# jbelyeu/unfazed

Hardware: AMD Instinct MI355X
Metric: phased DNMs/sec (higher is better)
Workload: dtype u8/int32 (+f64 allele balance); 1 GPU; 100k synthetic SNV/INDEL DNMs, whole-genome sites VCF, --no-extended off (BASELINE configs[2]); staged: H2D of the pre-decoded columns inside the timed region; dnms_per_gpu=100000, sites=20000000, coverage=30x, search_dist=5000, dnm_placement=uniform, read_clusters=67821, alignment_records=186931612, parallelism=dnm-shard x1, no collective

## Files before the change

### include/unfazed_io.h

```cpp
#ifndef UNFAZED_IO_H
#define UNFAZED_IO_H
#include <stdint.h>
#include "uz_types.h"
#include "uz_bamwalk.h"

#ifdef __cplusplus
extern "C" {
#endif

#define UZ_IO_OK 0
#define UZ_IO_E_OPEN (-1)
#define UZ_IO_E_FORMAT (-2)
#define UZ_IO_E_UNSORTED (-3)
#define UZ_IO_E_RANGE (-4)
#define UZ_IO_E_ARG (-5)

const char *uz_io_last_error(void);

typedef struct uz_bam uz_bam;

int uz_bam_decode(const char *path, int threads, uz_bam **out);
int uz_bam_decode_regions(const char *path, const char *bai_path, int64_t n_iv, const int32_t *tid, const int32_t *lo, const int32_t *hi,
                          int64_t head_records, int threads, uz_bam **out);
int uz_bam_decode_memory(const uint8_t *stream, int64_t n, int threads, uz_bam **out);
// ... 33 lines not shown
int uz_vcf_decode_regions(const char *path, const char *tbi_path, int64_t n_iv, const int32_t *ref, const int32_t *lo, const int32_t *hi,
                          int threads, uz_vcf **out);
int64_t uz_vcf_index_names(const char *path, const char *tbi_path, char *buf, int64_t cap);
int64_t uz_index_summary(const char *path, int kind, int64_t *out, int64_t cap_refs);
void uz_vcf_io_stats(const uz_vcf *h, int64_t out[4]);
void uz_vcf_free(uz_vcf *h);
int uz_vcf_view_get(const uz_vcf *h, uz_vcf_view *out);
const char *uz_vcf_sample(const uz_vcf *h, int32_t i);
const char *uz_vcf_contig(const uz_vcf *h, int32_t i);
const char *uz_vcf_ref(const uz_vcf *h, int64_t i, int32_t *len);
const char *uz_vcf_alt(const uz_vcf *h, int64_t i, int32_t *len);
const char *uz_vcf_header(const uz_vcf *h, int64_t *len);
const char *uz_vcf_line(const uz_vcf *h, int64_t i, int32_t *len);
const char *uz_vcf_info(const uz_vcf *h, int64_t i, const char *key, int32_t *len);
int uz_vcf_is_bcf(const uz_vcf *h);

int uz_reads_pack_sizes(const uz_reads_view *in, int64_t *n_cigar_total, int64_t *n_row_units);
int uz_reads_pack_cigar_omitted(const uz_reads_view *in, int threads, int64_t *n_omitted);
int uz_reads_pack_end_derivable(const uz_reads_view *in, int threads, int32_t *yes);
int uz_reads_pack_lists(const uz_reads_view *in, int min_base_qual, int threads, int64_t *n_qlow_pos, int32_t *wide);
int uz_reads_pack_exceptions(const uz_reads_view *in, int threads, int64_t *n_exc);
int uz_reads_pack(const uz_reads_view *in, int min_base_qual, int threads, uz_reads_packed_view *out);

typedef struct uz_psrc uz_psrc;
typedef struct uz_select uz_select;
int uz_reads_source_open(const uz_reads_packed_view *full, int threads, uz_psrc **out);
void uz_reads_source_close(uz_psrc *src);
int uz_reads_select_plan(const uz_psrc *src, int64_t n_fetch, const int32_t *contig, const int32_t *lo, const int32_t *hi, int all_bases,
                         int unit_masks, const uint16_t *extra, int tuples, int threads, uz_select **out);
int64_t uz_select_n_tuples(const uz_select *s);
// ... 82 lines not shown
```

### include/uz_types.h

```cpp
#ifndef UZ_TYPES_H
#define UZ_TYPES_H

#include <stdint.h>

#ifdef __cplusplus
extern "C" {
#endif

#define UZ_HOM_REF 0
#define UZ_HET 1
#define UZ_GT_UNKNOWN 2
#define UZ_HOM_ALT 3

#define UZ_U16_MISSING 0xFFFFu

#define UZ_SF_COMPLEX 1u

#define UZ_CL_HET 0x01u
#define UZ_CL_CAND 0x02u
#define UZ_CL_ALT_DAD 0x04u
#define UZ_CL_DEL_SHIFT 3
#define UZ_CL_DUP_SHIFT 5
#define UZ_KA_NONE 0
#define UZ_KA_REF_PARENT 1
// ... 48 lines not shown
    int32_t reserved0;
    double ab_homref[2];
    double ab_homalt[2];
    double ab_het[2];
} uz_params;

typedef struct uz_sites_view {
    int64_t n_sites;
    int32_t n_contigs;
    int32_t reserved0;
    const int64_t *contig_off;
    const int32_t *pos;
    const uint8_t *sflags;
    const uint8_t *ref_base;
    const uint8_t *alt_base;
} uz_sites_view;

typedef struct uz_family_view {
    const uint8_t *gt;
    const uint16_t *ref_depth[3];
    const uint16_t *alt_depth[3];
    const uint16_t *gq[3];
    int64_t n_wide;
    const int64_t *wide_site;
    const int32_t *wide_ref_depth[3];
    const int32_t *wide_alt_depth[3];
    const uint8_t *ref_depth8[3];
    const uint8_t *alt_depth8[3];
    const uint8_t *gq8[3];
} uz_family_view;
#define UZ_U8_MISSING 254u
// ... 153 lines not shown
```

### unfazed_amd/abi.py

```python
from __future__ import annotations

import ctypes as C
from typing import List, Optional, Sequence

import numpy as np

from .model import ReadsTable, SitesTable

ST_OK, ST_NO_CAND, ST_NO_OVERLAP, ST_REF_EXCEPTION, ST_SKIPPED, ST_CAPACITY = 0, 1, 2, 3, 4, 5
OR_NONE, OR_DAD, OR_MOM, OR_AMBIGUOUS = 0, 1, 2, 3
VT_POINT, VT_DEL, VT_DUP, VT_OTHER_SV = 0, 1, 2, 3
DF_FETCH_FALLBACK = 1
CF_ALT_DAD = 1
CF_KA_SHIFT = 1
CL_HET, CL_CAND, CL_ALT_DAD = 1, 2, 4
CL_DEL_SHIFT, CL_DUP_SHIFT = 3, 5
ET_READBACKED, ET_ALLELE_BALANCE, ET_AMBIGUOUS_READBACKED, ET_AMBIGUOUS_ALLELE_BALANCE, ET_AMBIGUOUS_BOTH, ET_AMBIG_FLAG = 1, 2, 4, 8, 16, 32
ET_NAMES = [(ET_READBACKED, "READBACKED"), (ET_AMBIGUOUS_READBACKED, "AMBIGUOUS_READBACKED"), (ET_ALLELE_BALANCE, "ALLELE-BALANCE"),
            (ET_AMBIGUOUS_ALLELE_BALANCE, "AMBIGUOUS_ALLELE-BALANCE"), (ET_AMBIGUOUS_BOTH, "AMBIGUOUS_BOTH")]
FIND_WHOLE_REGION = 1
FIND_SECOND_WINDOW = 2

_p = C.c_void_p

# ... 44 lines not shown
    p.ab_homalt[0], p.ab_homalt[1] = float(ab_homalt[0]), float(ab_homalt[1])
    p.ab_het[0], p.ab_het[1] = float(ab_het[0]), float(ab_het[1])
    return p


class SitesView(C.Structure):
    _fields_ = [
        ("n_sites", C.c_int64),
        ("n_contigs", C.c_int32),
        ("reserved0", C.c_int32),
        ("contig_off", _p),
        ("pos", _p),
        ("sflags", _p),
        ("ref_base", _p),
        ("alt_base", _p),
    ]


class FamilyView(C.Structure):
    _fields_ = [
        ("gt", _p),
        ("ref_depth", _p * 3),
        ("alt_depth", _p * 3),
        ("gq", _p * 3),
        ("n_wide", C.c_int64),
        ("wide_site", _p),
        ("wide_ref_depth", _p * 3),
        ("wide_alt_depth", _p * 3),
        ("ref_depth8", _p * 3),
        ("alt_depth8", _p * 3),
# ... 529 lines not shown
```

### unfazed_amd/csrc/abi.hip

```cpp
#include "uz_ctx.hpp"

#include <chrono>
#include <algorithm>
#include <map>
#include <mutex>

void uz_fold_complex(uz_ctx *c, uint8_t *gt, const uint8_t *sflags, int64_t n);
bool uz_site_scan_fresh(const uz_ctx *c, const FamilyDev &f, bool need_cnv);

namespace {

void set_error(uz_ctx *c, const std::string &msg) {
    std::lock_guard<std::mutex> lk(c->err_mu);
    c->err = msg;
}

template <typename F>
int guarded(uz_ctx *c, F &&fn) {
    if (!c) return UZ_E_ARG;
    try {
        (void)hipSetDevice(c->device);
        fn();
        return 0;
    } catch (const UzError &e) {
// ... 89 lines not shown
template <typename V>
int new_slot(std::vector<V> &v) {
    for (size_t i = 0; i < v.size(); i++)
        if (!v[i].live) return (int)i;
    v.emplace_back();
    return (int)v.size() - 1;
}

SitesDev &sites_of(uz_ctx *c, int id) {
    UZ_REQUIRE(id >= 0 && id < (int)c->sites.size() && c->sites[id].live, UZ_E_ARG, "unknown sites handle");
    SitesDev &s = c->sites[id];
    if (s.pending) {
        s.pending = false;
        UZ_HIP(hipStreamWaitEvent(c->stream, s.ready, 0));
    }
    return s;
}
FamilyDev &fam_of(uz_ctx *c, int id) {
    UZ_REQUIRE(id >= 0 && id < (int)c->fams.size() && c->fams[id].live, UZ_E_ARG, "unknown family handle");
    FamilyDev &f = c->fams[id];
    if (f.pending) {
        f.pending = false;
        UZ_HIP(hipStreamWaitEvent(c->stream, f.ready, 0));
        SitesDev &s = sites_of(c, f.sites_id);
        uz_family_widen(c, f, s.n);
        uz_fold_complex(c, f.gt, s.sflags, s.n);
    }
    return f;
}
ReadsDev &reads_of(uz_ctx *c, int id) {
    UZ_REQUIRE(id >= 0 && id < (int)c->reads.size() && c->reads[id].live, UZ_E_ARG, "unknown reads handle");
    return c->reads[id];
}

void free_family(uz_ctx *c, FamilyDev &f) {
    if (f.ready) { (void)hipEventSynchronize(f.ready); (void)hipEventDestroy(f.ready); f.ready = nullptr; }
    f.pending = false;
    uz_block_put(c, f.block);
    uz_block_put(c, f.wide_block);
    f = FamilyDev();
}
// ... 284 lines not shown

int uz_sync(uz_ctx *c) {
    return guarded(c, [&] { UZ_HIP(hipStreamSynchronize(c->stream)); });
}

int uz_set_params(uz_ctx *c, const uz_params *p) {
    return guarded(c, [&] {
        UZ_REQUIRE(p != nullptr, UZ_E_ARG, "null params");
        c->P = *p;
    });
}

int uz_sites_upload(uz_ctx *c, const uz_sites_view *v, int *id) {
    return guarded(c, [&] {
        UZ_REQUIRE(v && id && v->n_sites >= 0 && v->n_contigs >= 0, UZ_E_ARG, "bad sites view");
        UZ_REQUIRE(v->n_sites < (int64_t)0x7FFFFFF0, UZ_E_RANGE, "more than 2^31 sites");
        const int k = new_slot(c->sites);
        SitesDev s;
        s.live = true; s.owned = true;
        s.n = v->n_sites; s.n_contigs = v->n_contigs;
        s.contig_off_h.assign(v->contig_off, v->contig_off + v->n_contigs + 1);
        const size_t n = (size_t)s.n;
        for (int pass = 0; pass < 2; pass++) {
            Carver cv(pass ? s.block.p : nullptr);
            s.contig_off = cv.take<int64_t>((size_t)v->n_contigs + 1);
            s.pos = cv.take<int32_t>(n); s.sflags = cv.take<uint8_t>(n); s.ref_base = cv.take<uint8_t>(n); s.alt_base = cv.take<uint8_t>(n);
            if (!pass) s.block = uz_block_get(c, cv.off + 256);
        }
        try {
            h2d(c->stream, s.contig_off, v->contig_off, (size_t)v->n_contigs + 1);
            h2d(c->stream, s.pos, v->pos, n); h2d(c->stream, s.sflags, v->sflags, n);
            h2d(c->stream, s.ref_base, v->ref_base, n); h2d(c->stream, s.alt_base, v->alt_base, n);
            UZ_HIP(hipStreamSynchronize(c->stream));
        } catch (...) { uz_block_put(c, s.block); throw; }
        c->sites[k] = s;
        *id = k;
    });
}

int uz_sites_adopt_device(uz_ctx *c, const uz_sites_view *v, int *id) {
    return guarded(c, [&] {
        UZ_REQUIRE(v && id && v->n_sites >= 0 && v->n_contigs >= 0, UZ_E_ARG, "bad sites view");
        const int k = new_slot(c->sites);
        SitesDev s;
        s.live = true; s.owned = false;
        s.n = v->n_sites; s.n_contigs = v->n_contigs;
        s.contig_off_h.resize((size_t)v->n_contigs + 1);
        UZ_HIP(hipMemcpy(s.contig_off_h.data(), v->contig_off, ((size_t)v->n_contigs + 1) * sizeof(int64_t), hipMemcpyDeviceToHost));
        for (int pass = 0; pass < 2; pass++) {
            Carver cv(pass ? s.block.p : nullptr);
            s.contig_off = cv.take<int64_t>((size_t)v->n_contigs + 1);
            if (!pass) s.block = uz_block_get(c, cv.off + 256);
        }
        h2d(c->stream, s.contig_off, (const int64_t *)s.contig_off_h.data(), (size_t)v->n_contigs + 1);
        s.pos = const_cast<int32_t *>(v->pos);
        s.sflags = const_cast<uint8_t *>(v->sflags);
        s.ref_base = const_cast<uint8_t *>(v->ref_base);
        s.alt_base = const_cast<uint8_t *>(v->alt_base);
        UZ_HIP(hipStreamSynchronize(c->stream));
        c->sites[k] = s;
        *id = k;
    });
}

static bool family_view_eight(const uz_family_view *v) {
    int n8 = 0, n16 = 0;
    for (int m = 0; m < 3; m++) {
        n8 += (v->ref_depth8[m] != nullptr) + (v->alt_depth8[m] != nullptr) + (v->gq8[m] != nullptr);
        n16 += (v->ref_depth[m] != nullptr) + (v->alt_depth[m] != nullptr) + (v->gq[m] != nullptr);
    }
    UZ_REQUIRE((n8 == 9 && n16 == 0) || (n8 == 0 && n16 == 9) || (n8 == 0 && n16 == 0), UZ_E_ARG,
               "a family view carries its nine columns in 16 bits OR in 8 bits (ref_depth8 / alt_depth8 / gq8), all nine");
    return n8 == 9;
}

static void family_wide(uz_ctx *c, hipStream_t st, const uz_family_view *v, FamilyDev &f, int64_t n_sites) {
    f.n_wide = 0;
// ... 72 lines not shown
    });
}

int uz_sites_family_upload_async(uz_ctx *c, const uz_sites_view *v, const uz_family_view *fv, int *sites_id, int *fam_id) {
    return guarded(c, [&] {
        UZ_REQUIRE(v && fv && sites_id && fam_id && v->n_sites >= 0 && v->n_contigs >= 0, UZ_E_ARG, "bad sites / family view");
        UZ_REQUIRE(v->n_sites < (int64_t)0x7FFFFFF0, UZ_E_RANGE, "more than 2^31 sites");
        SitesDev s;
        s.live = true; s.owned = true;
        s.n = v->n_sites; s.n_contigs = v->n_contigs;
        s.contig_off_h.assign(v->contig_off, v->contig_off + v->n_contigs + 1);
        const size_t n = (size_t)s.n;
        FamilyDev f;
        f.owned = true;
        const bool eight = family_view_eight(fv);
        uint8_t *st8[9] = {nullptr, nullptr, nullptr, nullptr, nullptr, nullptr, nullptr, nullptr, nullptr};
        for (int pass = 0; pass < 2; pass++) {
            Carver cv(pass ? s.block.p : nullptr);
            s.contig_off = cv.take<int64_t>((size_t)v->n_contigs + 1);
            s.pos = cv.take<int32_t>(n); s.sflags = cv.take<uint8_t>(n); s.ref_base = cv.take<uint8_t>(n); s.alt_base = cv.take<uint8_t>(n);
            if (!pass) s.block = uz_block_get(c, cv.off + 256);
        }
        for (int pass = 0; pass < 2; pass++) {
            Carver cv(pass ? f.block.p : nullptr);
            f.cls = cv.take<uint8_t>(n);
            f.gt = cv.take<uint8_t>(n);
            for (int m = 0; m < 3; m++) { f.rd[m] = cv.take<uint16_t>(n); f.ad[m] = cv.take<uint16_t>(n); f.gq[m] = cv.take<uint16_t>(n); }
            if (eight) for (int k = 0; k < 9; k++) st8[k] = cv.take<uint8_t>(n);
            if (!pass) f.block = uz_block_get(c, cv.off + 256);
        }
        try {
            hipStream_t st = c->copy_stream;
            SlabPlan plan;
            SlabScope slab_scope(&plan);
            for (int stage_pass = 0; stage_pass < 2; stage_pass++) {
                if (stage_pass) slab_commit(c, st, plan, s.mirror);
                s.contig_off = const_cast<int64_t *>(h2d(st, s.contig_off, v->contig_off, (size_t)v->n_contigs + 1));
                s.pos = const_cast<int32_t *>(h2d(st, s.pos, v->pos, n)); s.sflags = const_cast<uint8_t *>(h2d(st, s.sflags, v->sflags, n));
                s.ref_base = const_cast<uint8_t *>(h2d(st, s.ref_base, v->ref_base, n)); s.alt_base = const_cast<uint8_t *>(h2d(st, s.alt_base, v->alt_base, n));
                f.gt = const_cast<uint8_t *>(h2d(st, f.gt, fv->gt, n));
                if (eight) {
                    for (int m = 0; m < 3; m++) {
                        f.stage8[m] = h2d(st, st8[m], fv->ref_depth8[m], n); f.stage8[3 + m] = h2d(st, st8[3 + m], fv->alt_depth8[m], n);
                        f.stage8[6 + m] = h2d(st, st8[6 + m], fv->gq8[m], n);
                    }
                } else
                    for (int m = 0; m < 3; m++) {
                        f.rd[m] = const_cast<uint16_t *>(h2d(st, f.rd[m], fv->ref_depth[m], n));
                        f.ad[m] = const_cast<uint16_t *>(h2d(st, f.ad[m], fv->alt_depth[m], n));
                        f.gq[m] = const_cast<uint16_t *>(h2d(st, f.gq[m], fv->gq[m], n));
                    }
            }
            if (eight) { f.widen_pending = true; f.gq_clamped = true; }
            family_wide(c, st, fv, f, s.n);
            UZ_HIP(hipEventCreateWithFlags(&f.ready, hipEventDisableTiming));
            UZ_HIP(hipEventRecord(f.ready, st));
            UZ_HIP(hipEventCreateWithFlags(&s.ready, hipEventDisableTiming));
            UZ_HIP(hipEventRecord(s.ready, st));
            s.pending = true;
        } catch (...) { uz_block_put(c, s.block); uz_block_put(c, s.mirror); uz_block_put(c, f.block); uz_block_put(c, f.wide_block); throw; }
        const int ks = new_slot(c->sites);
        c->sites[ks] = s;
        f.live = true; f.sites_id = ks; f.pending = true;
        const int kf = new_slot(c->fams);
        c->fams[kf] = f;
        *sites_id = ks; *fam_id = kf;
    });
}
// ... 1518 lines not shown
```

### unfazed_amd/csrc/io_vcf.cpp

```cpp
#include <map>
#include <memory>

#include "io_common.hpp"
#include "io_index.hpp"

#include <cmath>
#include <cstdlib>

using namespace uzio;

struct uz_vcf {
    Bytes text;
    std::vector<std::string> samples, contigs;
    std::string header;
    int64_t n = 0;
    std::vector<int64_t> contig_off;
    std::vector<int32_t> pos, end;
    std::vector<uint8_t> sflags, ref_base, alt_base;
    std::vector<uint8_t> gt;
    std::vector<int32_t> ref_depth, alt_depth;
    std::vector<double> gq;
    std::vector<uint64_t> line_at;
    std::vector<uint32_t> line_len, ref_at, ref_len, alt_at, alt_len;
    std::vector<uint32_t> chrom_len;
// ... 1044 lines not shown
        if ((size_t)(stop - q) > kl && memcmp(q, key, kl) == 0 && q[kl] == '=') { best = q + kl + 1; best_len = (int32_t)(stop - best); }
        else if ((size_t)(stop - q) == kl && memcmp(q, key, kl) == 0) { best = nullptr; best_len = 0; }
        if (!sc) break;
        q = sc + 1;
    }
    if (best && len) *len = best_len;
    return best;
}

const char *uz_vcf_line(const uz_vcf *h, int64_t i, int32_t *len) {
    if (!h || i < 0 || i >= h->n) return nullptr;
    if (len) *len = (int32_t)h->line_len[(size_t)i];
    return (const char *)h->text.data() + h->line_at[(size_t)i];
}

}
```

### unfazed_amd/csrc/k_sites.hip

```cpp
#include "uz_ctx.hpp"

#include <algorithm>
#include <cstdlib>
#include <vector>

namespace {

struct SiteParams {
    int32_t min_gt_qual, min_depth;
    double lo_ref, hi_ref, lo_het, hi_het, lo_alt, hi_alt;
};

__device__ __forceinline__ int dec16(uint32_t v) { return (int)(int16_t)(uint16_t)v; }

#define UZ_AB_T_MIN (-2)
#define UZ_AB_T_MAX 65534
#define UZ_AB_LUT_N (UZ_AB_T_MAX - UZ_AB_T_MIN + 1)
#define UZ_AB_A_MIN (-1)
#define UZ_AB_A_MAX 32767
__device__ __forceinline__ double ab_lo(const SiteParams &P, int gt) { return gt == UZ_HOM_REF ? P.lo_ref : (gt == UZ_HOM_ALT ? P.lo_alt : P.lo_het); }
__device__ __forceinline__ double ab_hi(const SiteParams &P, int gt) { return gt == UZ_HOM_REF ? P.hi_ref : (gt == UZ_HOM_ALT ? P.hi_alt : P.hi_het); }

#define UZ_AB_LDS_T 512
__global__ void k_build_ab_lut(SiteParams P, int2 *lut, uint32_t *small, int *t0_special) {
// ... 633 lines not shown
    for (int m = 0; m < 3; m++) {
        w.s[m] = f.stage8[m]; w.s[3 + m] = f.stage8[3 + m]; w.s[6 + m] = f.stage8[6 + m];
        w.d[m] = f.rd[m]; w.d[3 + m] = f.ad[m]; w.d[6 + m] = f.gq[m];
    }
    hipLaunchKernelGGL(k_widen8, dim3(nb), dim3(256), 0, c->stream, n, w);
    UZ_HIP(hipGetLastError());
}

void uz_fold_complex(uz_ctx *c, uint8_t *gt, const uint8_t *sflags, int64_t n) {
    if (n <= 0) return;
    const int64_t nb = (n + 255) / 256;
    hipLaunchKernelGGL(k_fold_complex, dim3((unsigned)nb), dim3(256), 0, c->stream, gt, sflags, n);
    UZ_HIP(hipGetLastError());
}

bool uz_site_scan_fresh(const uz_ctx *c, const FamilyDev &f, bool need_cnv) {
    return f.cls_valid && (f.cls_has_cnv || !need_cnv) && site_params_equal(f.cls_params, c->P);
}

#ifndef UZ_SITE_SPT
#define UZ_SITE_SPT 8
#endif

namespace {

void ensure_ab_lut(uz_ctx *c, const SiteParams &sp) {
    if (c->ab_lut_valid && site_params_equal(c->ab_lut_params, c->P)) return;
    c->ab_lut.ensure((size_t)4 * UZ_AB_LUT_N * 2 + 4 + 4 * UZ_AB_LDS_T);
    int *flag = c->ab_lut.p + (size_t)4 * UZ_AB_LUT_N * 2;
    UZ_HIP(hipMemsetAsync(flag, 0, sizeof(int), c->stream));
// ... 196 lines not shown
```

### unfazed_amd/csrc/uz_ctx.hpp

```cpp
#pragma once
#include <hip/hip_runtime.h>

#include <cstdint>
#include <cstring>
#include <mutex>
#include <string>
#include <memory>
#include <vector>

#include "unfazed_hip.h"
#include "uz_bamwalk.h"

struct UzError {
    int code;
    std::string msg;
};

#define UZ_HIP(call)                                                                                   \
    do {                                                                                               \
        hipError_t e__ = (call);                                                                       \
        if (e__ != hipSuccess)                                                                         \
            throw UzError{UZ_E_HIP, std::string(#call) + ": " + hipGetErrorString(e__)};               \
    } while (0)

// ... 58 lines not shown
    size_t cap = 0;
};

struct SitesDev {
    bool live = false, owned = false;
    DevBlock block;
    DevBlock mirror;
    int64_t n = 0;
    int32_t n_contigs = 0;
    std::vector<int64_t> contig_off_h;
    int64_t *contig_off = nullptr;
    int32_t *pos = nullptr;
    uint8_t *sflags = nullptr, *ref_base = nullptr, *alt_base = nullptr;
    hipEvent_t ready = nullptr;
    bool pending = false;
};

struct FamilyDev {
    bool live = false, owned = false;
    DevBlock block;
    int sites_id = -1;
    uint8_t *gt = nullptr;
    uint16_t *rd[3] = {nullptr, nullptr, nullptr};
    uint16_t *ad[3] = {nullptr, nullptr, nullptr};
    uint16_t *gq[3] = {nullptr, nullptr, nullptr};
    uint8_t *cls = nullptr;
    int64_t n_wide = 0;
    int64_t *wide_site = nullptr;
    int32_t *wide_depth = nullptr;
    DevBlock wide_block;
// ... 264 lines not shown
    const uint8_t *n_low = nullptr, *qlow_pos = nullptr;
    int32_t qpos_wide = 0;
    const unsigned long long *pk_sums = nullptr;
};
void uz_kcopy(uz_ctx *c, void *dst, const void *src, size_t bytes);
void uz_reads_make_ready(uz_ctx *c, ReadsDev &r);
size_t uz_rec_scratch_bytes(int64_t n);
void uz_build_records(uz_ctx *c, hipStream_t st, ReadsDev &r, const RecColumns &col, void *off_scratch);
void uz_pack_ascii_rows(uz_ctx *c, hipStream_t st, ReadsDev &r, const uint32_t *cigar_in, const uint32_t *cigar_off_in,
                        const uint8_t *seq_in, const uint32_t *sq_off16_in, uint32_t *cigar_out, uint8_t *seq4_out);
void uz_build_qlow(uz_ctx *c, hipStream_t st, ReadsDev &r, int min_base_qual);
void uz_concat_table(uz_ctx *c, hipStream_t st, ReadsDev &dst, const ReadsDev &src, int64_t rec_base, int64_t cigar_base, int64_t unit_base,
                     int64_t seq_base, uint32_t qname_base);
void uz_finish_table(uz_ctx *c, hipStream_t st, ReadsDev &r);
void uz_family_widen(uz_ctx *c, FamilyDev &f, int64_t n_sites);
void uz_launch_site_scan(uz_ctx *c, FamilyDev &f, const SitesDev &s, bool with_cnv);
void uz_launch_site_scan_many(uz_ctx *c, FamilyDev *const *fams, int n_fam, const SitesDev &s, bool with_cnv);
void uz_launch_find(uz_ctx *c, FamilyDev &f, const SitesDev &s, int mode, bool host_offsets = true);
void uz_stage_dnms(uz_ctx *c, const uz_dnms_view *d);
void uz_launch_cnv(uz_ctx *c, const SitesDev &s, const int32_t *rb_counts_dev, int32_t *cnv_counts, int32_t *cnv_pos, int32_t *origin,
                   int32_t *evidence, int32_t *etype);
void uz_launch_phase(uz_ctx *c, FamilyDev &f, const SitesDev &s, ReadsDev &r, int32_t *status, int32_t *counts,
                     int32_t *origin, int32_t *evidence, bool defer = false);
bool uz_finish_phase(uz_ctx *c, int32_t *status, int32_t *counts, int32_t *origin, int32_t *evidence);
void uz_launch_inflate(uz_ctx *c, hipStream_t st, int64_t n_blocks, const uint8_t *comp, int64_t comp_bytes_padded, const int64_t *in_off,
                       const int64_t *out_off, uint8_t *out, int32_t *cursor_and_err);
void uz_launch_bam_walk(uz_ctx *c, hipStream_t st, int n_tasks, const uint8_t *buf, const int64_t *blk_at, const int64_t *blk_coff, const int32_t *task,
                        const int64_t *span, const int32_t *reach, const int32_t *fetch, int64_t *count, const int64_t *first, int64_t *walked, int32_t *flags,
                        uz_walk_desc *out, int64_t *n_direct, int64_t *tab_first);
void uz_launch_desc_filter(uz_ctx *c, hipStream_t st, bool fill, int n_tasks, const uz_walk_desc *in, const int64_t *first, const int64_t *count,
// ... 26 lines not shown
```

### unfazed_amd/io_native.py

```python
from __future__ import annotations

import ctypes as C
import os
import time
from typing import List, Sequence

import numpy as np

from . import abi
from .model import ReadsTable, SitesTable

_HERE = os.path.dirname(os.path.abspath(__file__))
_LIB = None

IO_EXPORTS = [
    "uz_io_last_error", "uz_bam_decode", "uz_bam_free", "uz_bam_n_contigs", "uz_bam_contig_name",
    "uz_bam_contig_length", "uz_bam_n_file_records", "uz_bam_n_records", "uz_bam_view", "uz_bam_qname",
    "uz_bam_tlen_head", "uz_bam_timing", "uz_bam_decode_regions", "uz_bam_io_stats", "uz_vcf_decode", "uz_vcf_free", "uz_vcf_view_get", "uz_vcf_sample",
    "uz_vcf_contig", "uz_vcf_ref", "uz_vcf_alt", "uz_vcf_header", "uz_vcf_line", "uz_vcf_info", "uz_vcf_is_bcf",
    "uz_reads_pack_sizes", "uz_reads_pack_exceptions", "uz_reads_pack_lists", "uz_reads_pack_end_derivable", "uz_reads_pack_cigar_omitted", "uz_reads_pack", "uz_reads_source_open", "uz_reads_source_close", "uz_reads_select_plan",
    "uz_select_n_records", "uz_select_n_cigar_total", "uz_select_n_row_units", "uz_select_n_seq_units", "uz_select_n_bl", "uz_select_n_bl_units", "uz_select_bl_wide", "uz_select_n_exc", "uz_select_n_qlow_pos", "uz_select_qlow_pos_wide", "uz_select_end_derivable", "uz_select_n_cigar_omitted", "uz_select_n_tuples", "uz_select_n_esc16", "uz_select_n_esc16_start8", "uz_select_n_esc16_narrow8", "uz_select_pair8_ok", "uz_select_n_esc16_pair8", "uz_select_n_new_names", "uz_select_qname_map",
    "uz_reads_select_fill", "uz_select_free", "uz_vcf_decode_regions", "uz_vcf_index_names", "uz_vcf_io_stats",
    "uz_bam_decode_memory",
    "uz_bamsrc_open", "uz_bamsrc_close", "uz_bamsrc_n_contigs", "uz_bamsrc_contig_name", "uz_bamsrc_contig_length", "uz_bamsrc_tlen_head",
    "uz_index_summary", "uz_inflate_backend", "uz_io_default_threads", "uz_io_cpu_quota", "uz_bam_stage_plan", "uz_bam_stage_begin", "uz_bam_stage_finish", "uz_stage_gather_blocks", "uz_stage_set_inflated", "uz_stage_sizes", "uz_stage_io_stats", "uz_stage_timing", "uz_stage_fill", "uz_stage_qname", "uz_stage_qnames",
    "uz_stage_free", "uz_stage_walk_plan_sizes", "uz_stage_walk_plan", "uz_bam_stage_finish_desc", "uz_stage_kept_sizes", "uz_stage_kept", "uz_stage_walk_host", "uz_stage_kept_debug", "uz_stage_name_records", "uz_packed_block_sums", "uz_stage_merge_subtasks", "uz_bam_stage_finish_sub",
    "uz_stage_walk_flagged", "uz_stage_lookup", "uz_stage_extra", "uz_stage_n_lookup_tasks",
]


class VcfView(C.Structure):
    _fields_ = [
        ("n_sites", C.c_int64), ("n_samples", C.c_int32), ("n_contigs", C.c_int32),
        ("contig_off", C.c_void_p), ("pos", C.c_void_p), ("end", C.c_void_p), ("sflags", C.c_void_p),
        ("ref_base", C.c_void_p), ("alt_base", C.c_void_p), ("gt", C.c_void_p), ("ref_depth", C.c_void_p),
        ("alt_depth", C.c_void_p), ("gq", C.c_void_p),
    ]


def lib_path() -> str:
    return os.environ.get("UZ_IO_LIB", os.path.join(_HERE, "libunfazed_io.so"))

# ... 28 lines not shown
    lib.uz_bam_qname.restype = C.c_void_p
    lib.uz_bam_tlen_head.argtypes = [C.c_void_p, C.c_void_p, C.c_int64]
    lib.uz_bam_tlen_head.restype = C.c_int64
    lib.uz_bam_decode_memory.argtypes = [C.c_char_p, C.c_int64, C.c_int, C.POINTER(C.c_void_p)]
    lib.uz_bam_timing.argtypes = [C.c_void_p, C.POINTER(C.c_double)]
    lib.uz_bam_timing.restype = None
    lib.uz_vcf_decode.argtypes = [C.c_char_p, C.c_int, C.POINTER(C.c_void_p)]
    lib.uz_vcf_decode_regions.argtypes = [C.c_char_p, C.c_char_p, C.c_int64, C.c_void_p, C.c_void_p, C.c_void_p, C.c_int, C.POINTER(C.c_void_p)]
    lib.uz_vcf_index_names.argtypes = [C.c_char_p, C.c_char_p, C.c_void_p, C.c_int64]
    lib.uz_vcf_index_names.restype = C.c_int64
    lib.uz_vcf_io_stats.argtypes = [C.c_void_p, C.POINTER(C.c_int64)]
    lib.uz_vcf_io_stats.restype = None
    lib.uz_vcf_free.argtypes = [C.c_void_p]
    lib.uz_vcf_free.restype = None
    lib.uz_vcf_view_get.argtypes = [C.c_void_p, C.POINTER(VcfView)]
    lib.uz_vcf_sample.argtypes = [C.c_void_p, C.c_int32]
    lib.uz_vcf_sample.restype = C.c_char_p
    lib.uz_vcf_contig.argtypes = [C.c_void_p, C.c_int32]
    lib.uz_vcf_contig.restype = C.c_char_p
    for fn in (lib.uz_vcf_ref, lib.uz_vcf_alt, lib.uz_vcf_line):
        fn.argtypes = [C.c_void_p, C.c_int64, C.POINTER(C.c_int32)]
        fn.restype = C.c_void_p
    lib.uz_vcf_info.argtypes = [C.c_void_p, C.c_int64, C.c_char_p, C.POINTER(C.c_int32)]
    lib.uz_vcf_info.restype = C.c_void_p
    lib.uz_vcf_is_bcf.argtypes = [C.c_void_p]
    lib.uz_vcf_header.argtypes = [C.c_void_p, C.POINTER(C.c_int64)]
    lib.uz_vcf_header.restype = C.c_void_p
    lib.uz_reads_pack_sizes.argtypes = [C.c_void_p, C.POINTER(C.c_int64), C.POINTER(C.c_int64)]
    lib.uz_reads_pack_exceptions.argtypes = [C.c_void_p, C.c_int, C.POINTER(C.c_int64)]
    lib.uz_reads_pack_lists.argtypes = [C.c_void_p, C.c_int, C.c_int, C.POINTER(C.c_int64), C.POINTER(C.c_int32)]
# ... 70 lines not shown
    _LIB = lib
    return lib


class IoError(RuntimeError):
    def __init__(self, code: int, msg: str):
        super().__init__("%s (code %d)" % (msg, code))
        self.code = code


def _check(lib, rc: int) -> None:
    if rc != 0:
        raise IoError(rc, (lib.uz_io_last_error() or b"").decode(errors="replace"))


def read_bam_stream_table(stream: bytes, threads: int = 0, insert_size_max_sample: int = 1000000) -> ReadsTable:
    lib = load()
    hp = C.c_void_p()
    _check(lib, lib.uz_bam_decode_memory(stream, len(stream), int(threads), C.byref(hp)))
    return _table_from_handle(lib, _Handle(hp.value, lib.uz_bam_free), insert_size_max_sample)


def _arr(ptr, n: int, dtype) -> np.ndarray:
    dtype = np.dtype(dtype)
    if n <= 0 or not ptr:
        return np.zeros(0, dtype=dtype)
    buf = (C.c_char * (n * dtype.itemsize)).from_address(ptr)
    return np.frombuffer(buf, dtype=dtype, count=n)


# ... 721 lines not shown
```

Baseline: 11.05 million DNMs/s.

## Upload sites in a compact delta-coded form and expand them on the GPU

Adds a compact site encoding: 16-bit position deltas within 1024-site spans plus an escape list, and ref, alt and complex flag packed into one byte. The compact form is uploaded instead of the plain int32 and u8 columns, and a device kernel rebuilds pos, sflags and bases through a segmented scan, fused with the genotype complex fold and the 8-to-16-bit widening. This cuts the H2D bytes for the 20M-site table inside the timed region. The cost is an extra expand kernel, host packing work, and a larger device block, since both the compact and the expanded columns are allocated. The new path only runs if the caller passes a packed view, and the diff does not show the harness doing so.

```diff
diff --git a/include/unfazed_io.h b/include/unfazed_io.h
--- a/include/unfazed_io.h
+++ b/include/unfazed_io.h
@@ -71,6 +71,9 @@
 const char *uz_vcf_line(const uz_vcf *h, int64_t i, int32_t *len);
 const char *uz_vcf_info(const uz_vcf *h, int64_t i, const char *key, int32_t *len);
 int uz_vcf_is_bcf(const uz_vcf *h);
+
+int uz_sites_pack(const uz_sites_view *in, uint8_t *out, int64_t cap, uz_sites_view *view, int64_t *bytes);
+int uz_sites_unpack(const uz_sites_view *v, int32_t *pos, uint8_t *sflags, uint8_t *ref_base, uint8_t *alt_base);
 
 int uz_reads_pack_sizes(const uz_reads_view *in, int64_t *n_cigar_total, int64_t *n_row_units);
 int uz_reads_pack_cigar_omitted(const uz_reads_view *in, int threads, int64_t *n_omitted);
diff --git a/include/uz_types.h b/include/uz_types.h
--- a/include/uz_types.h
+++ b/include/uz_types.h
@@ -86,7 +86,18 @@
     const uint8_t *sflags;
     const uint8_t *ref_base;
     const uint8_t *alt_base;
+    const uint16_t *pos_d16;
+    const uint8_t *bases8;
+    const int32_t *span_pos;
+    int64_t n_pos_esc;
+    const int32_t *pos_esc_idx;
+    const int32_t *pos_esc_val;
+    const int32_t *pos_esc_off;
 } uz_sites_view;
+#define UZ_SITE_SPAN 1024
+#define UZ_POS_D16_LIMIT 32768
+#define UZ_BASE3_CODES "\0ACGTN"
+
 
 typedef struct uz_family_view {
     const uint8_t *gt;
diff --git a/unfazed_amd/abi.py b/unfazed_amd/abi.py
--- a/unfazed_amd/abi.py
+++ b/unfazed_amd/abi.py
@@ -82,6 +82,13 @@
         ("sflags", _p),
         ("ref_base", _p),
         ("alt_base", _p),
+        ("pos_d16", _p),
+        ("bases8", _p),
+        ("span_pos", _p),
+        ("n_pos_esc", C.c_int64),
+        ("pos_esc_idx", _p),
+        ("pos_esc_val", _p),
+        ("pos_esc_off", _p),
     ]
 
 
diff --git a/unfazed_amd/csrc/abi.hip b/unfazed_amd/csrc/abi.hip
--- a/unfazed_amd/csrc/abi.hip
+++ b/unfazed_amd/csrc/abi.hip
@@ -127,6 +127,7 @@
         s.pending = false;
         UZ_HIP(hipStreamWaitEvent(c->stream, s.ready, 0));
     }
+    uz_sites_expand(c, s, nullptr);
     return s;
 }
 FamilyDev &fam_of(uz_ctx *c, int id) {
@@ -135,9 +136,15 @@
     if (f.pending) {
         f.pending = false;
         UZ_HIP(hipStreamWaitEvent(c->stream, f.ready, 0));
-        SitesDev &s = sites_of(c, f.sites_id);
-        uz_family_widen(c, f, s.n);
-        uz_fold_complex(c, f.gt, s.sflags, s.n);
+        SitesDev &s0 = c->sites[f.sites_id];
+        if (s0.expand_pending) {
+            if (s0.pending) { s0.pending = false; UZ_HIP(hipStreamWaitEvent(c->stream, s0.ready, 0)); }
+            uz_sites_expand(c, s0, &f);
+        } else {
+            SitesDev &s = sites_of(c, f.sites_id);
+            uz_family_widen(c, f, s.n);
+            uz_fold_complex(c, f.gt, s.sflags, s.n);
+        }
     }
     return f;
 }
@@ -452,6 +459,7 @@
 int uz_sites_upload(uz_ctx *c, const uz_sites_view *v, int *id) {
     return guarded(c, [&] {
         UZ_REQUIRE(v && id && v->n_sites >= 0 && v->n_contigs >= 0, UZ_E_ARG, "bad sites view");
+        UZ_REQUIRE(!v->pos_d16 && !v->bases8, UZ_E_ARG, "the compact site form is taken by uz_sites_family_upload_async only");
         UZ_REQUIRE(v->n_sites < (int64_t)0x7FFFFFF0, UZ_E_RANGE, "more than 2^31 sites");
         const int k = new_slot(c->sites);
         SitesDev s;
@@ -479,6 +487,7 @@
 int uz_sites_adopt_device(uz_ctx *c, const uz_sites_view *v, int *id) {
     return guarded(c, [&] {
         UZ_REQUIRE(v && id && v->n_sites >= 0 && v->n_contigs >= 0, UZ_E_ARG, "bad sites view");
+        UZ_REQUIRE(!v->pos_d16 && !v->bases8, UZ_E_ARG, "the compact site form is taken by uz_sites_family_upload_async only");
         const int k = new_slot(c->sites);
         SitesDev s;
         s.live = true; s.owned = false;
@@ -499,6 +508,24 @@
         c->sites[k] = s;
         *id = k;
     });
+}
+
+static bool sites_view_compact(const uz_sites_view *v) {
+    if (!v->pos_d16 && !v->bases8) return false;
+    const int64_t n = v->n_sites, n_spans = (n + UZ_SITE_SPAN - 1) / UZ_SITE_SPAN;
+    UZ_REQUIRE(v->pos_d16 && v->bases8 && !v->pos && !v->sflags && !v->ref_base && !v->alt_base, UZ_E_ARG,
+               "a compact sites view sets pos_d16 and bases8 and leaves pos / sflags / ref_base / alt_base null");
+    UZ_REQUIRE(v->span_pos && v->pos_esc_off && v->n_pos_esc >= 0 && (v->n_pos_esc == 0 || (v->pos_esc_idx && v->pos_esc_val)), UZ_E_ARG,
+               "a compact sites view needs span_pos, pos_esc_off and its escape list");
+    UZ_REQUIRE(v->pos_esc_off[0] == 0 && v->pos_esc_off[n_spans] == v->n_pos_esc, UZ_E_ARG, "pos_esc_off does not cover the escape list");
+    for (int64_t sp = 0; sp < n_spans; sp++) {
+        const int64_t a = v->pos_esc_off[sp], b = v->pos_esc_off[sp + 1];
+        UZ_REQUIRE(a <= b, UZ_E_ARG, "pos_esc_off must ascend");
+        for (int64_t e = a; e < b; e++)
+            UZ_REQUIRE(v->pos_esc_idx[e] >= sp * UZ_SITE_SPAN && v->pos_esc_idx[e] < std::min(n, (sp + 1) * UZ_SITE_SPAN) &&
+                           (e == a || v->pos_esc_idx[e] > v->pos_esc_idx[e - 1]), UZ_E_ARG, "an escape outside its span, or out of order");
+    }
+    return true;
 }
 
 static bool family_view_eight(const uz_family_view *v) {
@@ -601,11 +628,20 @@
         FamilyDev f;
         f.owned = true;
         const bool eight = family_view_eight(fv);
+        const bool compact = sites_view_compact(v);
+        const size_t n_spans = (n + UZ_SITE_SPAN - 1) / UZ_SITE_SPAN, n_esc = compact ? (size_t)v->n_pos_esc : 0;
         uint8_t *st8[9] = {nullptr, nullptr, nullptr, nullptr, nullptr, nullptr, nullptr, nullptr, nullptr};
+        uint16_t *c_d16 = nullptr;
+        uint8_t *c_b8 = nullptr;
+        int32_t *c_span = nullptr, *c_eidx = nullptr, *c_eval = nullptr, *c_eoff = nullptr;
         for (int pass = 0; pass < 2; pass++) {
             Carver cv(pass ? s.block.p : nullptr);
             s.contig_off = cv.take<int64_t>((size_t)v->n_contigs + 1);
             s.pos = cv.take<int32_t>(n); s.sflags = cv.take<uint8_t>(n); s.ref_base = cv.take<uint8_t>(n); s.alt_base = cv.take<uint8_t>(n);
+            if (compact) {
+                c_d16 = cv.take<uint16_t>(n); c_b8 = cv.take<uint8_t>(n); c_span = cv.take<int32_t>(n_spans);
+                c_eidx = cv.take<int32_t>(n_esc); c_eval = cv.take<int32_t>(n_esc); c_eoff = cv.take<int32_t>(n_spans + 1);
+            }
             if (!pass) s.block = uz_block_get(c, cv.off + 256);
         }
         for (int pass = 0; pass < 2; pass++) {
@@ -623,8 +659,14 @@
             for (int stage_pass = 0; stage_pass < 2; stage_pass++) {
                 if (stage_pass) slab_commit(c, st, plan, s.mirror);
                 s.contig_off = const_cast<int64_t *>(h2d(st, s.contig_off, v->contig_off, (size_t)v->n_contigs + 1));
-                s.pos = const_cast<int32_t *>(h2d(st, s.pos, v->pos, n)); s.sflags = const_cast<uint8_t *>(h2d(st, s.sflags, v->sflags, n));
-                s.ref_base = const_cast<uint8_t *>(h2d(st, s.ref_base, v->ref_base, n)); s.alt_base = const_cast<uint8_t *>(h2d(st, s.alt_base, v->alt_base, n));
+                if (compact) {
+                    s.c_d16 = h2d(st, c_d16, v->pos_d16, n); s.c_b8 = h2d(st, c_b8, v->bases8, n); s.c_span = h2d(st, c_span, v->span_pos, n_spans);
+                    s.c_eidx = h2d(st, c_eidx, v->pos_esc_idx, n_esc); s.c_eval = h2d(st, c_eval, v->pos_esc_val, n_esc);
+                    s.c_eoff = h2d(st, c_eoff, v->pos_esc_off, n_spans + 1);
+                } else {
+                    s.pos = const_cast<int32_t *>(h2d(st, s.pos, v->pos, n)); s.sflags = const_cast<uint8_t *>(h2d(st, s.sflags, v->sflags, n));
+                    s.ref_base = const_cast<uint8_t *>(h2d(st, s.ref_base, v->ref_base, n)); s.alt_base = const_cast<uint8_t *>(h2d(st, s.alt_base, v->alt_base, n));
+                }
                 f.gt = const_cast<uint8_t *>(h2d(st, f.gt, fv->gt, n));
                 if (eight) {
                     for (int m = 0; m < 3; m++) {
@@ -639,6 +681,7 @@
                     }
             }
             if (eight) { f.widen_pending = true; f.gq_clamped = true; }
+            s.expand_pending = compact && n;
             family_wide(c, st, fv, f, s.n);
             UZ_HIP(hipEventCreateWithFlags(&f.ready, hipEventDisableTiming));
             UZ_HIP(hipEventRecord(f.ready, st));
diff --git a/unfazed_amd/csrc/io_vcf.cpp b/unfazed_amd/csrc/io_vcf.cpp
--- a/unfazed_amd/csrc/io_vcf.cpp
+++ b/unfazed_amd/csrc/io_vcf.cpp
@@ -1082,4 +1082,88 @@
     return (const char *)h->text.data() + h->line_at[(size_t)i];
 }
 
-}
+
+static int base3(uint8_t b) {
+    static const char codes[] = UZ_BASE3_CODES;
+    for (int k = 0; k < (int)sizeof(codes) - 1; k++)
+        if ((uint8_t)codes[k] == b) return k;
+    return -1;
+}
+
+int uz_sites_pack(const uz_sites_view *in, uint8_t *out, int64_t cap, uz_sites_view *view, int64_t *bytes) {
+    if (!in || !bytes || (out && !view)) { last_error = "null argument"; return UZ_IO_E_ARG; }
+    return guarded([&] {
+        const int64_t n = in->n_sites;
+        if (n < 0 || n >= ((int64_t)1 << 31) || in->n_contigs < 0) fail(UZ_IO_E_ARG, "bad site count");
+        if (n && (!in->pos || !in->sflags || !in->ref_base || !in->alt_base)) fail(UZ_IO_E_ARG, "uz_sites_pack takes the plain columns");
+        if (!in->contig_off) fail(UZ_IO_E_ARG, "null contig_off");
+        std::vector<uint8_t> first((size_t)n + 1, 0);
+        for (int32_t c = 0; c < in->n_contigs; c++) {
+            const int64_t a = in->contig_off[c], b = in->contig_off[c + 1];
+            if (a < 0 || b < a || b > n) fail(UZ_IO_E_ARG, "contig_off does not describe the table");
+            if (a < b) first[(size_t)a] = 1;
+        }
+        if (in->contig_off[0] != 0 || in->contig_off[in->n_contigs] != n) fail(UZ_IO_E_ARG, "contig_off does not describe the table");
+        const int64_t n_spans = (n + UZ_SITE_SPAN - 1) / UZ_SITE_SPAN;
+        auto escapes = [&](int64_t i) {
+            if (i % UZ_SITE_SPAN == 0) return false;
+            const int64_t d = (int64_t)in->pos[i] - in->pos[i - 1];
+            return first[(size_t)i] || d < 0 || d >= UZ_POS_D16_LIMIT;
+        };
+        int64_t n_esc = 0;
+        for (int64_t i = 0; i < n; i++) n_esc += escapes(i);
+        auto al = [](int64_t x) { return (x + 255) & ~(int64_t)255; };
+        const int64_t o_d16 = 0, o_b8 = al(o_d16 + 2 * n), o_span = al(o_b8 + n), o_idx = al(o_span + 4 * n_spans), o_val = al(o_idx + 4 * n_esc),
+                      o_off = al(o_val + 4 * n_esc), end = al(o_off + 4 * (n_spans + 1));
+        *bytes = end;
+        if (!out) return;
+        if (cap < end) fail(UZ_IO_E_ARG, "uz_sites_pack: %lld bytes of room for %lld", (long long)cap, (long long)end);
+        if ((uintptr_t)out % 256) fail(UZ_IO_E_ARG, "uz_sites_pack: the block must be 256-byte aligned");
+        uint16_t *d16 = (uint16_t *)(out + o_d16);
+        uint8_t *b8 = out + o_b8;
+        int32_t *span = (int32_t *)(out + o_span), *eidx = (int32_t *)(out + o_idx), *eval = (int32_t *)(out + o_val), *eoff = (int32_t *)(out + o_off);
+        int64_t e = 0;
+        for (int64_t i = 0; i < n; i++) {
+            const int r = base3(in->ref_base[i]), a = base3(in->alt_base[i]);
+            if (r < 0 || a < 0) fail(UZ_IO_E_RANGE, "site %lld: a base outside the three-bit codes", (long long)i);
+            if (in->sflags[i] & ~UZ_SF_COMPLEX) fail(UZ_IO_E_RANGE, "site %lld: a site flag the compact form does not carry", (long long)i);
+            b8[i] = (uint8_t)(r | a << 3 | (in->sflags[i] & UZ_SF_COMPLEX) << 6);
+            if (i % UZ_SITE_SPAN == 0) { span[i / UZ_SITE_SPAN] = in->pos[i]; eoff[i / UZ_SITE_SPAN] = (int32_t)e; }
+            if (escapes(i)) { eidx[e] = (int32_t)i; eval[e] = in->pos[i]; e++; d16[i] = 0; }
+            else d16[i] = (uint16_t)(i % UZ_SITE_SPAN ? in->pos[i] - in->pos[i - 1] : 0);
+        }
+        eoff[n_spans] = (int32_t)e;
+        memset(view, 0, sizeof(*view));
+        view->n_sites = n; view->n_contigs = in->n_contigs; view->contig_off = in->contig_off;
+        view->pos_d16 = d16; view->bases8 = b8; view->span_pos = span;
+        view->n_pos_esc = n_esc; view->pos_esc_idx = eidx; view->pos_esc_val = eval; view->pos_esc_off = eoff;
+    });
+}
+
+int uz_sites_unpack(const uz_sites_view *v, int32_t *pos, uint8_t *sflags, uint8_t *ref_base, uint8_t *alt_base) {
+    if (!v || !pos || !sflags || !ref_base || !alt_base) { last_error = "null argument"; return UZ_IO_E_ARG; }
+    return guarded([&] {
+        static const char codes[] = UZ_BASE3_CODES;
+        const int64_t n = v->n_sites, n_spans = (n + UZ_SITE_SPAN - 1) / UZ_SITE_SPAN;
+        if (n && (!v->pos_d16 || !v->bases8 || !v->span_pos || !v->pos_esc_off)) fail(UZ_IO_E_ARG, "not a compact site view");
+        for (int64_t s = 0; s < n_spans; s++) {
+            const int64_t lo = s * UZ_SITE_SPAN, hi = std::min(n, lo + UZ_SITE_SPAN);
+            int64_t e = v->pos_esc_off[s];
+            const int64_t e1 = v->pos_esc_off[s + 1];
+            if (e < 0 || e1 < e || e1 > v->n_pos_esc) fail(UZ_IO_E_ARG, "bad escape offsets");
+            uint32_t p = (uint32_t)v->span_pos[s];
+            for (int64_t i = lo; i < hi; i++) {
+                if (e < e1 && v->pos_esc_idx[e] == i) p = (uint32_t)v->pos_esc_val[e++];
+                else if (i > lo) p += v->pos_d16[i];
+                pos[i] = (int32_t)p;
+                const uint8_t b = v->bases8[i];
+                ref_base[i] = (uint8_t)codes[std::min(b & 7, 5)];
+                alt_base[i] = (uint8_t)codes[std::min(b >> 3 & 7, 5)];
+                sflags[i] = (uint8_t)(b >> 6 & 1);
+            }
+            if (e != e1) fail(UZ_IO_E_ARG, "span %lld: an escape outside its span", (long long)s);
+        }
+    });
+}
+
+}
diff --git a/unfazed_amd/csrc/k_sites.hip b/unfazed_amd/csrc/k_sites.hip
--- a/unfazed_amd/csrc/k_sites.hip
+++ b/unfazed_amd/csrc/k_sites.hip
@@ -671,6 +671,131 @@
     UZ_HIP(hipGetLastError());
 }
 
+struct SitesExpand {
+    const uint16_t *d16;
+    const uint8_t *b8;
+    const int32_t *span, *eidx, *eval, *eoff;
+    int32_t *pos;
+    uint8_t *sflags, *ref, *alt;
+    uint8_t *gt;
+    int widen;
+    Widen8 w;
+};
+__device__ __forceinline__ void seg_add(uint32_t &f, uint32_t &v, uint32_t fp, uint32_t vp) {
+    v = f ? v : vp + v;
+    f |= fp;
+}
+__global__ __launch_bounds__(256) void k_sites_expand(int64_t n, SitesExpand x) {
+    __shared__ uint16_t mark[UZ_SITE_SPAN];
+    __shared__ uint32_t wf[4], wv_[4];
+    const int t = threadIdx.x, lane = t & 63, wv = t >> 6;
+    const int64_t base = (int64_t)blockIdx.x * UZ_SITE_SPAN, i0 = base + 4 * t;
+    for (int j = t; j < UZ_SITE_SPAN; j += 256) mark[j] = 0;
+    __syncthreads();
+    const int32_t e0 = x.eoff[blockIdx.x], e1 = x.eoff[blockIdx.x + 1];
+    for (int32_t e = e0 + t; e < e1; e += 256) {
+        const int64_t l = (int64_t)x.eidx[e] - base;
+        if (l >= 0 && l < UZ_SITE_SPAN) mark[l] = (uint16_t)(e - e0 + 1);
+    }
+    __syncthreads();
+    const bool full = i0 + 3 < n;
+    uint32_t d[4] = {0, 0, 0, 0}, b[4] = {0, 0, 0, 0};
+    if (full) {
+        const ushort4 dv = *reinterpret_cast<const ushort4 *>(x.d16 + i0);
+        const uchar4 bv = *reinterpret_cast<const uchar4 *>(x.b8 + i0);
+        d[0] = dv.x; d[1] = dv.y; d[2] = dv.z; d[3] = dv.w;
+        b[0] = bv.x; b[1] = bv.y; b[2] = bv.z; b[3] = bv.w;
+    } else
+        for (int k = 0; k < 4; k++)
+            if (i0 + k < n) { d[k] = x.d16[i0 + k]; b[k] = x.b8[i0 + k]; }
+    uint32_t loc[4], locf[4], f = 0, acc = 0;
+#pragma unroll
+    for (int k = 0; k < 4; k++) {
+        const int l = 4 * t + k;
+        const uint32_t m = mark[l];
+        if (l == 0) { f = 1; acc = (uint32_t)x.span[blockIdx.x]; }
+        else if (m) { f = 1; acc = (uint32_t)x.eval[e0 + m - 1]; }
+        else acc += d[k];
+        loc[k] = acc; locf[k] = f;
+    }
+    uint32_t fi = f, vi = acc;
+#pragma unroll
+    for (int o = 1; o < 64; o <<= 1) {
+        const uint32_t fp = __shfl_up(fi, o, 64), vp = __shfl_up(vi, o, 64);
+        if (lane >= o) seg_add(fi, vi, fp, vp);
+    }
+    uint32_t fx = __shfl_up(fi, 1, 64), vx = __shfl_up(vi, 1, 64);
+    if (lane == 0) { fx = 0; vx = 0; }
+    if (lane == 63) { wf[wv] = fi; wv_[wv] = vi; }
+    __syncthreads();
+    uint32_t fp = 0, vp = 0;
+    for (int w = 0; w < wv; w++) { uint32_t fw = wf[w], vw = wv_[w]; seg_add(fw, vw, fp, vp); fp = fw; vp = vw; }
+    seg_add(fx, vx, fp, vp);
+    int32_t p[4];
+#pragma unroll
+    for (int k = 0; k < 4; k++) p[k] = (int32_t)(locf[k] ? loc[k] : vx + loc[k]);
+    const uint64_t codes = 0x4E4E4E54474341ull << 8;
+    uint8_t r8[4], a8[4], s8[4];
+#pragma unroll
+    for (int k = 0; k < 4; k++) {
+        r8[k] = (uint8_t)(codes >> (8 * (b[k] & 7u)));
+        a8[k] = (uint8_t)(codes >> (8 * (b[k] >> 3 & 7u)));
+        s8[k] = (uint8_t)(b[k] >> 6 & 1u);
+    }
+    if (full) {
+        *reinterpret_cast<int4 *>(x.pos + i0) = make_int4(p[0], p[1], p[2], p[3]);
+        *reinterpret_cast<uchar4 *>(x.ref + i0) = make_uchar4(r8[0], r8[1], r8[2], r8[3]);
+        *reinterpret_cast<uchar4 *>(x.alt + i0) = make_uchar4(a8[0], a8[1], a8[2], a8[3]);
+        *reinterpret_cast<uchar4 *>(x.sflags + i0) = make_uchar4(s8[0], s8[1], s8[2], s8[3]);
+        if (x.gt) {
+            const uchar4 g = *reinterpret_cast<const uchar4 *>(x.gt + i0);
+            *reinterpret_cast<uchar4 *>(x.gt + i0) = make_uchar4((uint8_t)((g.x & 0x3Fu) | (b[0] & 0x40u)), (uint8_t)((g.y & 0x3Fu) | (b[1] & 0x40u)),
+                                                               (uint8_t)((g.z & 0x3Fu) | (b[2] & 0x40u)), (uint8_t)((g.w & 0x3Fu) | (b[3] & 0x40u)));
+        }
+        if (x.widen) {
+#pragma unroll
+            for (int q = 0; q < 9; q++) {
+                const uchar4 v = *reinterpret_cast<const uchar4 *>(x.w.s[q] + i0);
+                const uint32_t miss = q < 6 ? (uint32_t)UZ_U8_MISSING : 255u;
+                auto wd = [&](uint32_t u) { return (uint16_t)(u == miss ? 0xFFFFu : u); };
+                *reinterpret_cast<ushort4 *>(x.w.d[q] + i0) = make_ushort4(wd(v.x), wd(v.y), wd(v.z), wd(v.w));
+            }
+        }
+        return;
+    }
+    for (int k = 0; k < 4; k++) {
+        const int64_t i = i0 + k;
+        if (i >= n) break;
+        x.pos[i] = p[k]; x.ref[i] = r8[k]; x.alt[i] = a8[k]; x.sflags[i] = s8[k];
+        if (x.gt) x.gt[i] = (uint8_t)((x.gt[i] & 0x3Fu) | (b[k] & 0x40u));
+        if (x.widen)
+            for (int q = 0; q < 9; q++) {
+                const uint32_t v = x.w.s[q][i];
+                x.w.d[q][i] = (uint16_t)(v == (q < 6 ? (uint32_t)UZ_U8_MISSING : 255u) ? 0xFFFFu : v);
+            }
+    }
+}
+void uz_sites_expand(uz_ctx *c, SitesDev &s, FamilyDev *f) {
+    if (!s.expand_pending) return;
+    s.expand_pending = false;
+    SitesExpand x{};
+    x.d16 = s.c_d16; x.b8 = s.c_b8; x.span = s.c_span; x.eidx = s.c_eidx; x.eval = s.c_eval; x.eoff = s.c_eoff;
+    x.pos = s.pos; x.sflags = s.sflags; x.ref = s.ref_base; x.alt = s.alt_base;
+    if (f) {
+        x.gt = f->gt;
+        x.widen = f->widen_pending;
+        f->widen_pending = false;
+        for (int m = 0; m < 3; m++) {
+            x.w.s[m] = f->stage8[m]; x.w.s[3 + m] = f->stage8[3 + m]; x.w.s[6 + m] = f->stage8[6 + m];
+            x.w.d[m] = f->rd[m]; x.w.d[3 + m] = f->ad[m]; x.w.d[6 + m] = f->gq[m];
+        }
+    }
+    if (s.n <= 0) return;
+    const unsigned nb = (unsigned)((s.n + UZ_SITE_SPAN - 1) / UZ_SITE_SPAN);
+    hipLaunchKernelGGL(k_sites_expand, dim3(nb), dim3(256), 0, c->stream, s.n, x);
+    UZ_HIP(hipGetLastError());
+}
+
 bool uz_site_scan_fresh(const uz_ctx *c, const FamilyDev &f, bool need_cnv) {
     return f.cls_valid && (f.cls_has_cnv || !need_cnv) && site_params_equal(f.cls_params, c->P);
 }
diff --git a/unfazed_amd/csrc/uz_ctx.hpp b/unfazed_amd/csrc/uz_ctx.hpp
--- a/unfazed_amd/csrc/uz_ctx.hpp
+++ b/unfazed_amd/csrc/uz_ctx.hpp
@@ -96,6 +96,10 @@
     uint8_t *sflags = nullptr, *ref_base = nullptr, *alt_base = nullptr;
     hipEvent_t ready = nullptr;
     bool pending = false;
+    bool expand_pending = false;
+    const uint16_t *c_d16 = nullptr;
+    const uint8_t *c_b8 = nullptr;
+    const int32_t *c_span = nullptr, *c_eidx = nullptr, *c_eval = nullptr, *c_eoff = nullptr;
 };
 
 struct FamilyDev {
@@ -390,6 +394,7 @@
                      int64_t seq_base, uint32_t qname_base);
 void uz_finish_table(uz_ctx *c, hipStream_t st, ReadsDev &r);
 void uz_family_widen(uz_ctx *c, FamilyDev &f, int64_t n_sites);
+void uz_sites_expand(uz_ctx *c, SitesDev &s, FamilyDev *f);
 void uz_launch_site_scan(uz_ctx *c, FamilyDev &f, const SitesDev &s, bool with_cnv);
 void uz_launch_site_scan_many(uz_ctx *c, FamilyDev *const *fams, int n_fam, const SitesDev &s, bool with_cnv);
 void uz_launch_find(uz_ctx *c, FamilyDev &f, const SitesDev &s, int mode, bool host_offsets = true);
diff --git a/unfazed_amd/io_native.py b/unfazed_amd/io_native.py
--- a/unfazed_amd/io_native.py
+++ b/unfazed_amd/io_native.py
@@ -25,7 +25,7 @@
     "uz_bamsrc_open", "uz_bamsrc_close", "uz_bamsrc_n_contigs", "uz_bamsrc_contig_name", "uz_bamsrc_contig_length", "uz_bamsrc_tlen_head",
     "uz_index_summary", "uz_inflate_backend", "uz_io_default_threads", "uz_io_cpu_quota", "uz_bam_stage_plan", "uz_bam_stage_begin", "uz_bam_stage_finish", "uz_stage_gather_blocks", "uz_stage_set_inflated", "uz_stage_sizes", "uz_stage_io_stats", "uz_stage_timing", "uz_stage_fill", "uz_stage_qname", "uz_stage_qnames",
     "uz_stage_free", "uz_stage_walk_plan_sizes", "uz_stage_walk_plan", "uz_bam_stage_finish_desc", "uz_stage_kept_sizes", "uz_stage_kept", "uz_stage_walk_host", "uz_stage_kept_debug", "uz_stage_name_records", "uz_packed_block_sums", "uz_stage_merge_subtasks", "uz_bam_stage_finish_sub",
-    "uz_stage_walk_flagged", "uz_stage_lookup", "uz_stage_extra", "uz_stage_n_lookup_tasks",
+    "uz_stage_walk_flagged", "uz_stage_lookup", "uz_stage_extra", "uz_stage_n_lookup_tasks", "uz_sites_pack", "uz_sites_unpack",
 ]
 
 
@@ -84,6 +84,8 @@
     lib.uz_vcf_free.argtypes = [C.c_void_p]
     lib.uz_vcf_free.restype = None
     lib.uz_vcf_view_get.argtypes = [C.c_void_p, C.POINTER(VcfView)]
+    lib.uz_sites_pack.argtypes = [C.POINTER(abi.SitesView), C.c_void_p, C.c_int64, C.POINTER(abi.SitesView), C.POINTER(C.c_int64)]
+    lib.uz_sites_unpack.argtypes = [C.POINTER(abi.SitesView), C.c_void_p, C.c_void_p, C.c_void_p, C.c_void_p]
     lib.uz_vcf_sample.argtypes = [C.c_void_p, C.c_int32]
     lib.uz_vcf_sample.restype = C.c_char_p
     lib.uz_vcf_contig.argtypes = [C.c_void_p, C.c_int32]
@@ -184,6 +186,30 @@
         raise IoError(rc, (lib.uz_io_last_error() or b"").decode(errors="replace"))
 
 
+def pack_sites(plain: "abi.SitesView", alloc=None):
+    lib = load()
+    nb = C.c_int64(0)
+    _check(lib, lib.uz_sites_pack(C.byref(plain), None, 0, None, C.byref(nb)))
+    size = max(256, int(nb.value))
+    if alloc is None:
+        raw = np.zeros(size + 256, np.uint8)
+        k = (-raw.ctypes.data) % 256
+        block = raw[k: k + size]
+    else:
+        block = alloc(size)
+    v = abi.SitesView()
+    _check(lib, lib.uz_sites_pack(C.byref(plain), block.ctypes.data, int(block.nbytes), C.byref(v), C.byref(nb)))
+    return v, block, int(nb.value)
+
+
+def unpack_sites(v: "abi.SitesView"):
+    lib = load()
+    n = int(v.n_sites)
+    pos, sf, rb, ab = np.zeros(n + 1, np.int32), np.zeros(n + 1, np.uint8), np.zeros(n + 1, np.uint8), np.zeros(n + 1, np.uint8)
+    _check(lib, lib.uz_sites_unpack(C.byref(v), pos.ctypes.data, sf.ctypes.data, rb.ctypes.data, ab.ctypes.data))
+    return pos[:n], sf[:n], rb[:n], ab[:n]
+
+
 def read_bam_stream_table(stream: bytes, threads: int = 0, insert_size_max_sample: int = 1000000) -> ReadsTable:
     lib = load()
     hp = C.c_void_p()
```

Result: faster. 11.62 million DNMs/s, median of 6 (+5.1%).
